# arpg/Kangaroo

Measured on AMD Instinct MI355X. Metric: kinectfusion_frames_per_sec_640x480_to_512cubed_tsdf, higher is better.
Workload: dtype f32

## Files before the change

kangaroo_amd/csrc/kfx_device.h:

```cpp
#pragma once

#include <hip/hip_runtime.h>
#include <stddef.h>
#include <stdint.h>

#include "../../include/kfx.h"
#include "../../include/kfx_extras.h"
#include "../../include/kfx_summary_h.h"
#include "../../include/kfx_color.h"
#include "summary_ring_host.h"

namespace kfx {

struct V3 { float x, y, z; };

__device__ __forceinline__ V3 v3(float x, float y, float z) { return V3{x, y, z}; }
__device__ __forceinline__ V3 operator+(V3 a, V3 b) { return V3{a.x + b.x, a.y + b.y, a.z + b.z}; }
__device__ __forceinline__ V3 operator-(V3 a, V3 b) { return V3{a.x - b.x, a.y - b.y, a.z - b.z}; }
__device__ __forceinline__ V3 operator*(V3 a, float s) { return V3{a.x * s, a.y * s, a.z * s}; }
__device__ __forceinline__ V3 div_cw(V3 a, V3 b) { return V3{a.x / b.x, a.y / b.y, a.z / b.z}; }
__device__ __forceinline__ V3 div_s(V3 a, float s) { const float inv = 1.0f / s; return a * inv; }
__device__ __forceinline__ float dot(V3 a, V3 b) { return a.x * b.x + a.y * b.y + a.z * b.z; }
__device__ __forceinline__ float length(V3 a) { return sqrtf(dot(a, a)); }
__device__ __forceinline__ float lerp(float a, float b, float t) { return a + t * (b - a); }
// ... 224 lines not shown
                all_either = all_either && c != 0;
            }
            cls = all_free ? 1 : (all_nan ? 2 : (all_either ? 3 : 0));
        }
        const unsigned long long p0 = __ballot(cls & 1), p1 = __ballot(cls & 2);
        if (e < total && (bx & 63) == 0 && (chunks > 1 || bx == 0)) {
            const int sh = chunks > 1 ? 0 : lane;
            const unsigned long long m = (chunks > 1 || lg == 6) ? ~0ull : ((1ull << (1 << lg)) - 1ull);
            const unsigned long long r0 = (p0 >> sh) & m, r1 = (p1 >> sh) & m;
            unsigned* out = tab + dst.first + (bz * dst.ny + by) * dst.rw + (bx >> 6) * 4;
            out[0] = (unsigned)r0; out[1] = (unsigned)r1;
            if ((bx >> 6) * 4 + 2 < dst.rw) { out[2] = (unsigned)(r0 >> 32); out[3] = (unsigned)(r1 >> 32); }
        }
    }
}
int summary_classes_prepare(kfx_sdf_summary* s, float tol, float vref, int fine_shift, hipStream_t stream, int global = 0);
void summary_class_layout(const kfx_sdf_summary* s, int fine_shift, ClassView& cv);
void summary_top_layout(const ClassView& cv, ClassLevel& l6, ClassLevel& l7, int& w6, int& w7);
int summary_view_offset(const kfx_sdf_summary* s, const kfx_volume* view, int* ox, int* oy, int* oz);
}

namespace kfx {
int set_error(int code, const char* what);
int check_launch(const char* what);
int hip_status(hipError_t e, const char* what);
int math_mode();
size_t texel_image_bytes(size_t w, size_t h);
int depth_to_vbo_normals_texels(const kfx_image* vbo, const kfx_image* nrm, const kfx_image* depth, const float K[4], float scale,
                                const kfx_image* texels, kfx_stream stream);
int sdf_fuse_slab_texels(const kfx_volume* vol, const kfx_slab* slab, const kfx_image* depth, const kfx_image* norm, const kfx_image* texels,
                         const float T_cw[12], const float K[4], float trunc_dist, float max_w, float mincostheta, unsigned flags, kfx_stream stream);
// ... 4 lines not shown
```

kangaroo_amd/csrc/raycast.hip:

```cpp
#include <cmath>
#include <thread>

#include <hip/hip_fp16.h>

#include "kfx_device.h"
#include "sampling.h"
#include "../../include/kfx_slab_color.h"

namespace kfx {

struct RayParams {
    VolView vol;
    V3 size;
    V3 dims1;
    V3 hi2;
    V3 voxel;
    V3 inv_size;
    int fastdiv, off32;
    Pose T;
    Intr K;
    unsigned char *dptr, *nptr, *iptr;
    size_t dpitch, npitch, ipitch;
    int w, h;
    float near, far, trunc;
// ... 353 lines not shown
    const int at = GT ? 0 : cl.words;
    class_level_up(cl.nx5, cl.coarse.ny, cl.nz5, 6, at, l6, nx6, nz6, w6);
    class_level_up(nx6, l6.ny, nz6, 7, at + w6, l7, nx7, nz7, w7);
    if (threadIdx.x == 0) { top.lv[0] = l6; top.lv[1] = l7; top.n = cl.top_n; }
    __syncthreads();
}

__device__ __forceinline__ bool workgroup_any(const bool yes, int* s_any)
{
    const bool wave_any = __ballot(yes) != 0ull;
    if ((threadIdx.x & 63) == 0) s_any[threadIdx.x >> 6] = wave_any ? 1 : 0;
    __syncthreads();
    return (s_any[0] | s_any[1] | s_any[2] | s_any[3]) != 0;
}

template <typename CELL, bool GT = false>
__global__ __launch_bounds__(256) void k_raycast_sdf_classes(const RayParams p, const ClassView cl)
{
    extern __shared__ unsigned s_tab[];
    __shared__ RayParams s_p;
    __shared__ TopLevels s_top;
    __shared__ int s_any[4];
    if (threadIdx.x == 0) s_p = p;
    int u, v;
    const bool carries = ray_lane_pixel(p, p.sparse_lanes, blockIdx.x, blockIdx.y, u, v);
    const bool pixel = carries && u < p.w && v < p.h;
    if constexpr (!GT) {
        if (!workgroup_any(pixel && enters(ray_box(p, u, v)), s_any)) {
            if (pixel) write_no_hit(ray_out(p, u, v));
            return;
        }
    }
    classes_stage<GT>(cl, s_tab, s_top);
    if (!carries) return;
    raycast_pixel_classes<CELL, false, false, GT>(p, s_p, ColorGeom{}, u, v, cl, s_tab, s_top);
}

template <typename CELL, bool COLOR>
__global__ __launch_bounds__(256) void k_raycast_sdf(const RayParams p, const ColorGeom cv)
{
    int u, v;
    if (!ray_lane_pixel(p, p.sparse_lanes, blockIdx.x, blockIdx.y, u, v)) return;
    raycast_pixel<CELL, COLOR>(p, cv, u, v);
}

template <typename CELL>
__global__ __launch_bounds__(256) void k_raycast_sdf_count(const RayParams p, unsigned* __restrict__ bitmap, unsigned long long* __restrict__ counters)
{
    int u, v;
    ray_pixel_of(p, blockIdx.x, blockIdx.y, threadIdx.x, u, v);
// ... 305 lines not shown
    p.npitch = norm->pitch;
    p.ipitch = img->pitch;
    p.w = (int)img->w;
    p.h = (int)img->h;
    p.near = near;
    p.far = far;
    p.trunc = trunc_dist;
    p.subpix = subpix ? 1 : 0;
    p.tile_log2w = 5;
    p.wg_log2x = 1;
    p.sparse_lanes = 0;
    return 0;
}

template <typename CELL>
static int class_view(ClassView& cl, size_t* lds_bytes, int* usable, kfx_sdf_summary* summary, const kfx_volume* vol, const RayParams& p, kfx_stream stream,
                      bool allow_global = true)
{
    *usable = 0;
    if (int e = summary_view_offset(summary, vol, &cl.ox, &cl.oy, &cl.oz)) return e;
    if (!(p.trunc > 0.f) || !(p.trunc < __builtin_inff())) return 0;
    static const int kb_env = env_int("KFX_RAYCAST_CLASS_KB", 16, 1, 60);
    static const int gt_env = env_int("KFX_RAYCAST_GLOBAL_TABLES", 0);
    static const int top_env = env_int("KFX_RAYCAST_TOP_LEVELS", 2, 0, 2);
    int fine = 3;
    for (; fine < 5; ++fine) {
        summary_class_layout(summary, fine, cl);
        if ((size_t)cl.words * 4 <= (size_t)kb_env * 1024) break;
    }
    auto top_levels = [&](int& w6, int& w7) {
        summary_class_layout(summary, fine, cl);
        cl.nx5 = ceil_div(summary->w, 32); cl.nz5 = ceil_div(summary->d, 32);
        ClassLevel l6, l7;
        summary_top_layout(cl, l6, l7, w6, w7);
// ... 14 lines not shown
        cl.top_first = cl.words;
        cl.lds_words = (cl.top_n > 0 ? w6 : 0) + (cl.top_n > 1 ? w7 : 0);
        if ((size_t)cl.lds_words * 4 + lds_static > 64 * 1024) return 0;
    } else {
        cl.top_first = 0;
        cl.lds_words = cl.words + derived;
    }
    if (cl.global && !allow_global) return 0;
    const bool half = CELL::BYTES == 4;
    const float vref = half ? __half2float(__float2half_rn(p.trunc)) : p.trunc;
    const float tol = math_mode() == KFX_MATH_FAST ? (half ? KFX_SUMMARY_HALF_BAND : 1e-5f) : 0.f;
    static const int force_env = env_int("KFX_RAYCAST_SUMMARY", 0);
    if (force_env < 0) return 0;
    const bool steer = force_env == 0 && summary->h_skippable;
    if (steer && summary->plain_calls && (summary->plain_calls++ % 8u) != 0u) return 0;
    if (int e = summary_classes_prepare(summary, tol, vref, fine, (hipStream_t)stream, cl.global)) return e;
    if (steer && summary->builds >= 3) {
        const unsigned ref = summary->builds - 3;
        const unsigned long long* slot = summary->h_skippable + summary_ring_index(ref);
        int known = 0;
        const int seen = summary_ring_wait(
            ref, 1ull << 20,
            [&]() {
                const uint64_t v = __atomic_load_n(slot, __ATOMIC_ACQUIRE);
                if (summary_ring_slot_stamp(v) != summary_ring_stamp(ref)) std::this_thread::yield();
                return v;
            },
            [&]() { (void)hipStreamSynchronize((hipStream_t)stream); }, &known);
        if (seen < 0) return set_error(KFX_E_TIMEOUT, "RaycastSdf(tracked): the class-table build the choice of the march rests on has not published its count");
        if ((long long)known * 4 < summary->n_coarse) {
            if (!summary->plain_calls) summary->plain_calls = 1;
// ... 13 lines not shown
    for (int a = 0; a < 3; ++a) {
        if (!(size[a] > 0.f)) return 0;
        const double sc = (double)dims1[a] / size[a];
        const double pmax = std::fmax(std::fabs((double)bmin[a]), std::fabs((double)bmax[a])), ca = std::fabs((double)cw[a]);
        const double A = std::fabs(((double)cw[a] - bmin[a]) * sc);
        const double t = sc * (3.0 * pmax + 2.0 * ca + size[a]) * u24 + 2.0 * dims1[a] * u24;
        const double e = u24 * (3.0 * A + 2.0 * sc * (pmax + ca) + dims1[a]) + 3.0 * u24 * (dims1[a] + A);
        eps = std::fmax(eps, t + e);
    }
    eps *= 2.0;
    if (!(eps < 0.05)) return 0;
    cl.eps = (float)std::fmax(eps, 1e-4);
    *lds_bytes = (size_t)cl.lds_words * sizeof(unsigned);
    *usable = 1;
    return 0;
}

template <typename PLAIN, typename... A>
static int launch_march(const char* what, int usable, const ClassView& cl, size_t cl_bytes, dim3 grid, kfx_stream stream, const RayParams& p,
                        void (*global)(RayParams, ClassView, A...), void (*lds)(RayParams, ClassView, A...), PLAIN plain, A... a)
{
    if (usable) hipLaunchKernelGGL(cl.global ? global : lds, grid, dim3(256), cl_bytes, (hipStream_t)stream, p, cl, a...);
    else plain();
    return check_launch(what);
}

template <typename CELL>
static int raycast_levels_launch(int n_levels, const kfx_image* const* depth, const kfx_image* const* norm, const kfx_image* const* img,
                                 const kfx_image* const* vbo, const kfx_volume* vol, const float T_wc[12], const float* K, float near, float far,
                                 float trunc_dist, int subpix, kfx_stream stream, kfx_sdf_summary* summary = nullptr)
// ... 64 lines not shown
    static const int lanes_env = [] { const int v = env_int("KFX_RAYCAST_LANES", 0); return (v == 8 || v == 16 || v == 32) ? v : (v < 0 ? -1 : 0); }();
    const int lanes = lanes_env ? lanes_env : ((long long)p.w * p.h <= 160 * 120 ? 16 : 0);
    if (lanes && lanes_env >= 0) {
        p.sparse_lanes = lanes;
        grid = dim3(ceil_div(p.w, 2 * lanes), ceil_div(p.h, 2));
    }
    ColorGeom cv{};
    if (colorvol) {
        if (int e = check_volume(colorvol, 4, 2, VOLUME_ANY_DIM, "RaycastSdf(colour)")) return e;
        set_geometry(cv, colorvol);
        hipLaunchKernelGGL((k_raycast_sdf<CELL, true>), grid, dim3(256), 0, (hipStream_t)stream, p, cv);
    } else if (summary) {
        ClassView cl;
        size_t cl_bytes = 0;
        int usable = 0;
        if (int e = class_view<CELL>(cl, &cl_bytes, &usable, summary, vol, p, stream)) return e;
        return launch_march("kfx_raycast_sdf_tracked", usable, cl, cl_bytes, grid, stream, p, k_raycast_sdf_classes<CELL, true>, k_raycast_sdf_classes<CELL, false>,
                            [&] { hipLaunchKernelGGL((k_raycast_sdf<CELL, false>), grid, dim3(256), 0, (hipStream_t)stream, p, cv); });
    } else {
        hipLaunchKernelGGL((k_raycast_sdf<CELL, false>), grid, dim3(256), 0, (hipStream_t)stream, p, cv);
    }
    return check_launch("kfx_raycast_sdf");
}

extern "C" int kfx_raycast_sdf(const kfx_image* depth, const kfx_image* norm, const kfx_image* img,
                               const kfx_volume* vol, const float T_wc[12], const float K[4], float near,
                               float far, float trunc_dist, int subpix, kfx_stream stream)
{
    return raycast_launch<RayF32>(depth, norm, img, vol, T_wc, K, near, far, trunc_dist, subpix, stream);
}

template <typename CELL>
static int count_params(RayParams& p, dim3& grid, const kfx_volume* vol, unsigned w, unsigned h, const float T_wc[12], const float K[4], float near, float far,
// ... 307 lines not shown
```

kangaroo_amd/csrc/summary.hip:

```cpp
#include <algorithm>
#include <new>

#include <hip/hip_fp16.h>

#include "kfx_device.h"

namespace kfx {

__global__ __launch_bounds__(256) void k_summary_fill(float4* __restrict__ R, size_t n, float lo, float hi, int state)
{
    const size_t i = (size_t)blockIdx.x * 256 + threadIdx.x;
    if (i < n) R[i] = make_float4(lo, hi, __int_as_float(state), 0.f);
}

struct ClassBuild {
    const float4* R;
    unsigned* C;
    int nbx, nby, nbz;
    int shift, nx, ny, nz, rw;
    float lo_ok, hi_ok;
    const unsigned* src;
    int src_shift, src_nx, src_ny, src_nz, src_rw;
};
struct TopBuild {
    int on;
    unsigned* tab;
    ClassLevel l5, l6, l7;
    int nx5, nz5, nx6, nz6, nx7, nz7;
};
template <int M>
__device__ __forceinline__ int class_row(const ClassBuild& b, const long long wave)
{
    const float4* __restrict__ R = b.R;
    unsigned* __restrict__ C = b.C;
    const unsigned* __restrict__ src = b.src;
    const int nbx = b.nbx, nby = b.nby, nbz = b.nbz, shift = b.shift, nx = b.nx, ny = b.ny, rw = b.rw;
    const int src_shift = b.src_shift, src_nx = b.src_nx, src_ny = b.src_ny, src_nz = b.src_nz, src_rw = b.src_rw;
    const float lo_ok = b.lo_ok, hi_ok = b.hi_ok;
    const int lane = threadIdx.x & 63;
    const int chunks = (nx + 63) >> 6;
    const int chunk = (int)(wave % chunks), by = (int)((wave / chunks) % ny), bz = (int)(wave / ((long long)chunks * ny));
    const int bx = chunk * 64 + lane;
    int cls = 0;
    if (bx < nx) {
        bool all_nan = true, all_free = true, all_either = true;
        if constexpr (M == 0) {
            const int m = 1 << (shift - src_shift);
            for (int z0 = 0; z0 < m; z0 += 2) {
                uint2 w2[2][4];
#pragma unroll
                for (int dz = 0; dz < 2; ++dz)
#pragma unroll
                    for (int dy = 0; dy < 4; ++dy) {
                        const int z = min(bz * m + z0 + dz, src_nz - 1), y = min(by * m + min(dy, m - 1), src_ny - 1);
                        w2[dz][dy] = *reinterpret_cast<const uint2*>(src + ((size_t)z * src_ny + y) * src_rw + (((bx * m) >> 5) << 1));
                    }
#pragma unroll
                for (int dz = 0; dz < 2; ++dz)
#pragma unroll
                    for (int dy = 0; dy < 4; ++dy)
                        for (int dx = 0; dx < m; ++dx) {
                            const int x = min(bx * m + dx, src_nx - 1);
                            const int c = (int)((w2[dz][dy].x >> (x & 31)) & 1u) | (int)(((w2[dz][dy].y >> (x & 31)) & 1u) << 1);
                            all_free = all_free && c == 1;
                            all_nan = all_nan && c == 2;
                            all_either = all_either && c != 0;
                        }
            }
        } else if constexpr (M > 2) {
#pragma unroll 1
            for (int z = bz * M; z <= bz * M + M; ++z)
#pragma unroll 1
                for (int y = by * M; y <= by * M + M; ++y) {
                    const float4* __restrict__ Rrow = R + ((size_t)min(z, nbz - 1) * nby + min(y, nby - 1)) * nbx;
                    float4 r[M + 1];
#pragma unroll
                    for (int dx = 0; dx <= M; ++dx) r[dx] = Rrow[min(bx * M + dx, nbx - 1)];
#pragma unroll
                    for (int dx = 0; dx <= M; ++dx) {
                        const unsigned m = brick_class_mask(r[dx].x, r[dx].y, __float_as_int(r[dx].z), lo_ok, hi_ok);
                        all_nan = all_nan && (m & 1u);
                        all_free = all_free && (m & 2u);
                        all_either = all_either && (m & 4u);
                    }
                }
        } else {
            float4 r[(M + 1) * (M + 1) * (M + 1)];
#pragma unroll
            for (int dz = 0; dz <= M; ++dz)
#pragma unroll
                for (int dy = 0; dy <= M; ++dy)
#pragma unroll
                    for (int dx = 0; dx <= M; ++dx)
                        r[(dz * (M + 1) + dy) * (M + 1) + dx] =
                            R[((size_t)min(bz * M + dz, nbz - 1) * nby + min(by * M + dy, nby - 1)) * nbx + min(bx * M + dx, nbx - 1)];
#pragma unroll
            for (int k = 0; k < (M + 1) * (M + 1) * (M + 1); ++k) {
                const unsigned m = brick_class_mask(r[k].x, r[k].y, __float_as_int(r[k].z), lo_ok, hi_ok);
                all_nan = all_nan && (m & 1u);
                all_free = all_free && (m & 2u);
                all_either = all_either && (m & 4u);
            }
        }
        cls = all_free ? 1 : (all_nan ? 2 : (all_either ? 3 : 0));
    }
    const unsigned long long p0 = __ballot(cls & 1), p1 = __ballot(cls & 2);
    if (lane == 0) {
        unsigned* row = C + ((size_t)bz * ny + by) * rw + chunk * 4;
        row[0] = (unsigned)p0; row[1] = (unsigned)p1;
        if (chunk * 4 + 2 < rw) { row[2] = (unsigned)(p0 >> 32); row[3] = (unsigned)(p1 >> 32); }
    }
    return __popcll(p0 | p1);
}

__device__ __forceinline__ bool classes_up_to_date(int* __restrict__ count, unsigned long long* __restrict__ publish, const unsigned stamp,
                                                   const int* __restrict__ dirty, const int conditional)
{
    if (!conditional || *dirty != 0) return false;
    if (blockIdx.x == 0 && threadIdx.x == 0) {
        __hip_atomic_store(publish, ((unsigned long long)stamp << 32) | (unsigned)count[2], __ATOMIC_RELAXED, __HIP_MEMORY_SCOPE_SYSTEM);
        count[4] += 1;
    }
    return true;
}

__device__ __forceinline__ void classes_count_and_top(const int n, int* __restrict__ count, unsigned long long* __restrict__ publish, const unsigned stamp,
                                                      int* __restrict__ dirty, const int conditional, const TopBuild& t)
{
    __shared__ int s_count[4];
    __shared__ int s_last;
    if ((threadIdx.x & 63) == 0) s_count[threadIdx.x >> 6] = n;
    __threadfence();
    __syncthreads();
    if (threadIdx.x == 0) {
        s_last = 0;
        atomicAdd(&count[0], s_count[0] + s_count[1] + s_count[2] + s_count[3]);
        __threadfence();
        if (atomicAdd(&count[1], 1) == (int)gridDim.x - 1) {
            __threadfence();
            s_last = 1;
            const int total = atomicExch(&count[0], 0);
            count[1] = 0;
            count[2] = total;
            if (conditional) count[3] += 1;
            *dirty = 0;
            __hip_atomic_store(publish, ((unsigned long long)stamp << 32) | (unsigned)total, __ATOMIC_RELAXED, __HIP_MEMORY_SCOPE_SYSTEM);
        }
    }
    __syncthreads();
    if (t.on && s_last) {
        __threadfence();
        classes_level_up(t.tab, t.l5, t.nx5, t.nz5, t.l6, t.nx6, t.nz6);
        __threadfence();
        __syncthreads();
        classes_level_up(t.tab, t.l6, t.nx6, t.nz6, t.l7, t.nx7, t.nz7);
    }
}

struct FineRows {
    unsigned* C;
    int shift, nx, ny, nz, rw;
    int blocks;
    long long waves;
};
template <int MF>
__global__ __launch_bounds__(256) void k_summary_classes_build(const FineRows f, const ClassBuild c, const long long c_waves, int* __restrict__ count,
                                                               unsigned long long* __restrict__ publish, const unsigned stamp, int* __restrict__ dirty,
                                                               const int conditional, const TopBuild t)
{
    if (classes_up_to_date(count, publish, stamp, dirty, conditional)) return;
    int n = 0;
    bool fine_row = false;
    if constexpr (MF != 0) {
        fine_row = (int)blockIdx.x < f.blocks;
        if (fine_row) {
            ClassBuild b = c;
            b.C = f.C; b.shift = f.shift; b.nx = f.nx; b.ny = f.ny; b.nz = f.nz; b.rw = f.rw;
            const long long wave = (long long)blockIdx.x * 4 + (threadIdx.x >> 6);
            if (wave < f.waves) class_row<MF>(b, wave);
        }
    }
    if (!fine_row) {
        const long long wave = (long long)((int)blockIdx.x - f.blocks) * 4 + (threadIdx.x >> 6);
        if (wave < c_waves) n = class_row<4>(c, wave);
    }
    classes_count_and_top(n, count, publish, stamp, dirty, conditional, t);
}

template <int M>
__global__ __launch_bounds__(256) void k_summary_classes(const ClassBuild b, const long long n_waves)
{
    const long long wave = (long long)blockIdx.x * 4 + (threadIdx.x >> 6);
    if (wave < n_waves) class_row<M>(b, wave);
}

__global__ __launch_bounds__(256) void k_summary_classes_coarse(const ClassBuild b, const long long n_waves, int* __restrict__ count,
                                                                unsigned long long* __restrict__ publish, const unsigned stamp, int* __restrict__ dirty, const TopBuild t)
{
    const long long wave = (long long)blockIdx.x * 4 + (threadIdx.x >> 6);
    const int n = wave < n_waves ? class_row<0>(b, wave) : 0;
    classes_count_and_top(n, count, publish, stamp, dirty, 0, t);
}

template <int BYTES>
__global__ __launch_bounds__(256) void k_summary_rebuild(float4* __restrict__ R, const unsigned char* __restrict__ base, size_t pitch, size_t img_pitch,
                                                         int w, int h, int d, int nbx, int nby, int nbz, int aligned16)
{
    const long long brick = (long long)blockIdx.x * 4 + (threadIdx.x >> 6);
    if (brick >= (long long)nbx * nby * nbz) return;
    const int lane = threadIdx.x & 63;
    const int bx = (int)(brick % nbx), by = (int)((brick / nbx) % nby), bz = (int)(brick / ((long long)nbx * nby));
    const int y = by * 8 + (lane & 7), z = bz * 8 + (lane >> 3), x0 = bx * 8;
    float lo = __builtin_inff(), hi = -__builtin_inff();
    bool nan = false, val = false;
    if (y < h && z < d) {
        const unsigned char* row = base + (size_t)z * img_pitch + (size_t)y * pitch + (size_t)x0 * BYTES;
// ... 61 lines not shown
void summary_class_layout(const kfx_sdf_summary* s, int fine_shift, ClassView& cv)
{
    class_level(cv.fine, fine_shift, s->w, s->h, 0);
    const int fw = fine_shift < 5 ? class_level_words(cv.fine, s->d) : 0;
    class_level(cv.coarse, 5, s->w, s->h, (fw + 3) & ~3);
    cv.words = cv.coarse.first + ((class_level_words(cv.coarse, s->d) + 3) & ~3);
}

void summary_top_layout(const ClassView& cv, ClassLevel& l6, ClassLevel& l7, int& w6, int& w7)
{
    int nx6, nz6, nx7, nz7;
    class_level_up(cv.nx5, cv.coarse.ny, cv.nz5, 6, cv.words, l6, nx6, nz6, w6);
    class_level_up(nx6, l6.ny, nz6, 7, cv.words + w6, l7, nx7, nz7, w7);
}

int summary_classes_prepare(kfx_sdf_summary* s, float tol, float vref, int fine_shift, hipStream_t stream, int global)
{
    const bool same = s->c_tol == tol && s->c_vref == vref && s->c_shift == fine_shift && s->c_global == global;
    if (!s->c_dirty && same) return 0;
    const int conditional = (s->c_dirty == 1 && same && !global) ? 1 : 0;
    ClassView cv;
    summary_class_layout(s, fine_shift, cv);
    cv.nx5 = ceil_div(s->w, 32); cv.nz5 = ceil_div(s->d, 32);
    ClassLevel l6, l7;
    int w6, w7;
    summary_top_layout(cv, l6, l7, w6, w7);
    TopBuild top{};
    top.on = global ? 0 : 1;
    top.tab = s->C;
    top.l5 = cv.coarse; top.l6 = l6; top.l7 = l7;
    top.nx5 = cv.nx5; top.nz5 = cv.nz5;
    top.nx6 = (top.nx5 + 1) >> 1; top.nz6 = (top.nz5 + 1) >> 1;
// ... 19 lines not shown
    if (global && has_fine) {
        const ClassBuild f = level(cv.fine, nullptr), c = level(cv.coarse, &cv.fine);
        if (cv.fine.shift == 3) hipLaunchKernelGGL(k_summary_classes<1>, dim3(blocks_of(f)), dim3(256), 0, stream, f, waves_of(f));
        else hipLaunchKernelGGL(k_summary_classes<2>, dim3(blocks_of(f)), dim3(256), 0, stream, f, waves_of(f));
        if (int e = launched()) return e;
        hipLaunchKernelGGL(k_summary_classes_coarse, dim3(blocks_of(c)), dim3(256), 0, stream, c, waves_of(c), s->d_count, publish, stamp, s->d_dirty, top);
        if (int e = launched()) return e;
    } else {
        const ClassBuild c = level(cv.coarse, nullptr);
        FineRows f{};
        if (has_fine) {
            const ClassBuild b = level(cv.fine, nullptr);
            f.C = b.C; f.shift = b.shift; f.nx = b.nx; f.ny = b.ny; f.nz = b.nz; f.rw = b.rw;
            f.blocks = (int)blocks_of(b); f.waves = waves_of(b);
        }
        const dim3 grid((unsigned)f.blocks + blocks_of(c));
        if (!has_fine) hipLaunchKernelGGL(k_summary_classes_build<0>, grid, dim3(256), 0, stream, f, c, waves_of(c), s->d_count, publish, stamp, s->d_dirty, conditional, top);
        else if (cv.fine.shift == 3) hipLaunchKernelGGL(k_summary_classes_build<1>, grid, dim3(256), 0, stream, f, c, waves_of(c), s->d_count, publish, stamp, s->d_dirty, conditional, top);
        else hipLaunchKernelGGL(k_summary_classes_build<2>, grid, dim3(256), 0, stream, f, c, waves_of(c), s->d_count, publish, stamp, s->d_dirty, conditional, top);
        if (int e = launched()) return e;
    }
    s->builds += 1;
    if (global) {
        for (int up = 0; up < 2; ++up) {
            const ClassBuild b = level(up ? l7 : l6, up ? &l6 : &cv.coarse);
            hipLaunchKernelGGL(k_summary_classes<0>, dim3(blocks_of(b)), dim3(256), 0, stream, b, waves_of(b));
            if (int e = launched()) return e;
        }
    }
    s->c_dirty = 0; s->c_tol = tol; s->c_vref = vref; s->c_shift = fine_shift; s->c_global = global;
    s->c_lo_ok = lo_ok; s->c_hi_ok = hi_ok;
    return 0;
}

int summary_view_offset(const kfx_sdf_summary* s, const kfx_volume* view, int* ox, int* oy, int* oz)
// ... 31 lines not shown
    s->keep_stride = 0; s->keep_row0 = 0; s->keep_rows = 0;
    s->c_lo_ok = 0.f; s->c_hi_ok = 0.f; s->d_dirty = nullptr;
    s->builds = 0; s->plain_calls = 0; s->launches = 0;
    s->n_coarse = ceil_div(s->w, 32) * ceil_div(s->h, 32) * ceil_div(s->d, 32);
    const size_t n = (size_t)s->nbx * s->nby * s->nbz;
    ClassView cv;
    summary_class_layout(s, 3, cv);
    cv.nx5 = ceil_div(s->w, 32); cv.nz5 = ceil_div(s->d, 32);
    ClassLevel l6, l7;
    int w6, w7;
    summary_top_layout(cv, l6, l7, w6, w7);
    const int words = cv.words + w6 + w7;
    bool ok = hipMalloc((void**)&s->R, n * sizeof(float4)) == hipSuccess && hipMalloc((void**)&s->C, (size_t)words * sizeof(unsigned)) == hipSuccess &&
              hipMalloc((void**)&s->d_count, 64 * sizeof(int)) == hipSuccess && hipMemset(s->d_count, 0, 64 * sizeof(int)) == hipSuccess;
    if (ok) s->d_dirty = s->d_count + 32;
    if (ok && hipHostMalloc((void**)&s->h_skippable, KFX_SUMMARY_RING * sizeof(unsigned long long), hipHostMallocMapped) == hipSuccess) {
        for (int i = 0; i < KFX_SUMMARY_RING; ++i) s->h_skippable[i] = 0ull;
        if (hipHostGetDevicePointer((void**)&s->d_skippable, s->h_skippable, 0) != hipSuccess) {
            (void)hipHostFree(s->h_skippable);
            s->h_skippable = nullptr;
        }
    } else {
        s->h_skippable = nullptr;
    }
    if (ok && !s->h_skippable) {
        (void)hipGetLastError();
        ok = hipMalloc((void**)&s->d_skippable, sizeof(unsigned long long)) == hipSuccess;
    }
    if (!ok) {
        (void)hipGetLastError();
        kfx_sdf_summary_destroy(s);
        return set_error(KFX_E_NODEVICE, "kfx_sdf_summary_create: hipMalloc");
    }
    *out = s;
    return kfx_sdf_summary_invalidate(s, nullptr);
}

extern "C" int kfx_sdf_summary_create(kfx_sdf_summary** out, const kfx_volume* vol) { return summary_create(out, vol, 8); }
extern "C" int kfx_sdf_summary_create_h(kfx_sdf_summary** out, const kfx_volume* vol) { return summary_create(out, vol, 4); }

extern "C" int kfx_sdf_summary_destroy(kfx_sdf_summary* s)
{
    if (!s) return 0;
    (void)hipDeviceSynchronize();
    if (s->R) (void)hipFree(s->R);
    if (s->C) (void)hipFree(s->C);
    if (s->d_count) (void)hipFree(s->d_count);
    if (s->h_skippable) (void)hipHostFree(s->h_skippable);
    else if (s->d_skippable) (void)hipFree(s->d_skippable);
    delete s;
    return 0;
}

extern "C" int kfx_sdf_summary_rebuild(kfx_sdf_summary* s, kfx_stream stream)
{
    if (!s) return set_error(KFX_E_NULL, "kfx_sdf_summary_rebuild: null summary");
    const long long n = (long long)s->nbx * s->nby * s->nbz;
    const int aligned16 = ((((uintptr_t)s->base) | s->pitch | s->img_pitch) & 15) == 0;
    if (s->cell_bytes == 4)
        hipLaunchKernelGGL(k_summary_rebuild<4>, dim3((unsigned)((n + 3) / 4)), dim3(256), 0, (hipStream_t)stream, s->R, s->base, s->pitch, s->img_pitch,
                           s->w, s->h, s->d, s->nbx, s->nby, s->nbz, aligned16);
    else
        hipLaunchKernelGGL(k_summary_rebuild<8>, dim3((unsigned)((n + 3) / 4)), dim3(256), 0, (hipStream_t)stream, s->R, s->base, s->pitch, s->img_pitch,
                           s->w, s->h, s->d, s->nbx, s->nby, s->nbz, aligned16);
    s->c_dirty = 2;
    return check_launch("kfx_sdf_summary_rebuild");
}

extern "C" int kfx_sdf_summary_invalidate(kfx_sdf_summary* s, kfx_stream stream)
{
    if (!s) return set_error(KFX_E_NULL, "kfx_sdf_summary_invalidate: null summary");
    const size_t n = (size_t)s->nbx * s->nby * s->nbz;
    hipLaunchKernelGGL(k_summary_fill, dim3((unsigned)((n + 255) / 256)), dim3(256), 0, (hipStream_t)stream, s->R, n, -__builtin_inff(), __builtin_inff(), 2);
    s->c_dirty = 2;
    return check_launch("kfx_sdf_summary_invalidate");
}

static int reset_tracked(const kfx_volume* vol, kfx_sdf_summary* s, float trunc_dist, kfx_stream stream, int cell_bytes, const char* name)
{
    if (!s) return set_error(KFX_E_NULL, cell_bytes == 4 ? "kfx_sdf_reset_tracked_h: null summary" : "kfx_sdf_reset_tracked: null summary");
    if (s->cell_bytes != cell_bytes) return set_error(KFX_E_SHAPE, "SdfReset(tracked): the summary was created for the other cell type");
    int ox, oy, oz;
    if (int e = summary_view_offset(s, vol, &ox, &oy, &oz)) return e;
    if (ox || oy || oz || (int)vol->w != s->w || (int)vol->h != s->h || (int)vol->d != s->d)
        return set_error(KFX_E_SHAPE, "kfx_sdf_reset_tracked: resets the whole volume only (use kfx_sdf_reset + kfx_sdf_summary_invalidate for views)");
    if (int e = cell_bytes == 4 ? kfx_sdf_reset_h(vol, trunc_dist, stream) : kfx_sdf_reset(vol, trunc_dist, stream)) return e;
    const size_t n = (size_t)s->nbx * s->nby * s->nbz;
    const bool nan = trunc_dist != trunc_dist;
    const float v = cell_bytes == 4 ? __half2float(__float2half_rn(trunc_dist)) : trunc_dist;
    hipLaunchKernelGGL(k_summary_fill, dim3((unsigned)((n + 255) / 256)), dim3(256), 0, (hipStream_t)stream, s->R, n,
                       nan ? __builtin_inff() : v, nan ? -__builtin_inff() : v, nan ? 1 : 0);
    s->c_dirty = 2;
    return check_launch(name);
}

extern "C" int kfx_sdf_reset_tracked(const kfx_volume* vol, kfx_sdf_summary* s, float trunc_dist, kfx_stream stream)
// ... 9 lines not shown
```

Measured before the change: 2637.

## Fuse class-table build into the tracked raycast launch via ticketed work-sharing

```diff
diff --git a/kangaroo_amd/csrc/kfx_device.h b/kangaroo_amd/csrc/kfx_device.h
--- a/kangaroo_amd/csrc/kfx_device.h
+++ b/kangaroo_amd/csrc/kfx_device.h
@@ -262,7 +262,10 @@
         }
     }
 }
-int summary_classes_prepare(kfx_sdf_summary* s, float tol, float vref, int fine_shift, hipStream_t stream, int global = 0);
+struct ClassRide;
+int summary_classes_prepare(kfx_sdf_summary* s, float tol, float vref, int fine_shift, hipStream_t stream, int global = 0, ClassRide* ride = nullptr);
+int summary_classes_launch(kfx_sdf_summary* s, const ClassRide& b, int conditional, hipStream_t stream, bool counted);
+int summary_ride_error(kfx_sdf_summary* s);
 void summary_class_layout(const kfx_sdf_summary* s, int fine_shift, ClassView& cv);
 void summary_top_layout(const ClassView& cv, ClassLevel& l6, ClassLevel& l7, int& w6, int& w7);
 int summary_view_offset(const kfx_sdf_summary* s, const kfx_volume* view, int* ox, int* oy, int* oz);
diff --git a/kangaroo_amd/csrc/raycast.hip b/kangaroo_amd/csrc/raycast.hip
--- a/kangaroo_amd/csrc/raycast.hip
+++ b/kangaroo_amd/csrc/raycast.hip
@@ -4,6 +4,7 @@
 #include <hip/hip_fp16.h>
 
 #include "kfx_device.h"
+#include "summary_build.h"
 #include "sampling.h"
 #include "../../include/kfx_slab_color.h"
 
@@ -391,13 +392,18 @@
     return (s_any[0] | s_any[1] | s_any[2] | s_any[3]) != 0;
 }
 
-template <typename CELL, bool GT = false>
-__global__ __launch_bounds__(256) void k_raycast_sdf_classes(const RayParams p, const ClassView cl)
-{
-    extern __shared__ unsigned s_tab[];
-    __shared__ RayParams s_p;
-    __shared__ TopLevels s_top;
-    __shared__ int s_any[4];
+struct ClassesArgs { RayParams p; ClassView cl; ClassRide rb; };
+typedef const __attribute__((address_space(4))) ClassesArgs* ClassesArgsPtr;
+__device__ __forceinline__ ClassesArgsPtr classes_args()
+{
+    ClassesArgsPtr a = (ClassesArgsPtr)__builtin_amdgcn_kernarg_segment_ptr();
+    asm volatile("" : "+s"(a));
+    return a;
+}
+
+template <typename CELL, bool GT>
+__device__ __forceinline__ void march_classes(const RayParams& p, const ClassView& cl, unsigned* s_tab, RayParams& s_p, TopLevels& s_top, int* s_any)
+{
     if (threadIdx.x == 0) s_p = p;
     int u, v;
     const bool carries = ray_lane_pixel(p, p.sparse_lanes, blockIdx.x, blockIdx.y, u, v);
@@ -411,6 +417,37 @@
     classes_stage<GT>(cl, s_tab, s_top);
     if (!carries) return;
     raycast_pixel_classes<CELL, false, false, GT>(p, s_p, ColorGeom{}, u, v, cl, s_tab, s_top);
+}
+
+template <typename CELL, bool GT = false>
+__global__ __launch_bounds__(256) void k_raycast_sdf_classes(const RayParams p, const ClassView cl, const ClassRide rb)
+{
+    extern __shared__ unsigned s_tab[];
+    __shared__ RayParams s_p;
+    __shared__ TopLevels s_top;
+    __shared__ int s_any[4];
+    if constexpr (GT) {
+        march_classes<CELL, true>(p, cl, s_tab, s_p, s_top, s_any);
+    } else {
+        if (rb.on) {
+            __shared__ int s_ride[2];
+            const int d = __builtin_amdgcn_readfirstlane(__hip_atomic_load(rb.dirty, __ATOMIC_RELAXED, __HIP_MEMORY_SCOPE_AGENT));
+            if (d == CLASSES_DIRTY || d == classes_built_mark(rb.stamp)) {
+                ClassesArgsPtr a = classes_args();
+                if (!classes_ride(*(const ClassRide*)&a->rb, s_ride)) {
+                    const RayParams& q = *(const RayParams*)&a->p;
+                    int u, v;
+                    if (ray_lane_pixel(q, q.sparse_lanes, blockIdx.x, blockIdx.y, u, v)) raycast_pixel<CELL, false>(q, ColorGeom{}, u, v);
+                    return;
+                }
+            } else if (blockIdx.x == 0 && blockIdx.y == 0 && threadIdx.x == 0) {
+                ClassesArgsPtr a = classes_args();
+                classes_publish_retained(a->rb.count, a->rb.publish, rb.stamp);
+            }
+        }
+        ClassesArgsPtr a = classes_args();
+        march_classes<CELL, false>(*(const RayParams*)&a->p, *(const ClassView*)&a->cl, s_tab, s_p, s_top, s_any);
+    }
 }
 
 template <typename CELL, bool COLOR>
@@ -746,10 +783,11 @@
 }
 
 template <typename CELL>
-static int class_view(ClassView& cl, size_t* lds_bytes, int* usable, kfx_sdf_summary* summary, const kfx_volume* vol, const RayParams& p, kfx_stream stream,
-                      bool allow_global = true)
+static int class_view_tables(ClassView& cl, size_t* lds_bytes, int* usable, kfx_sdf_summary* summary, const kfx_volume* vol, const RayParams& p, kfx_stream stream,
+                             bool allow_global, ClassRide* ride)
 {
     *usable = 0;
+    if (int e = summary_ride_error(summary)) return e;
     if (int e = summary_view_offset(summary, vol, &cl.ox, &cl.oy, &cl.oz)) return e;
     if (!(p.trunc > 0.f) || !(p.trunc < __builtin_inff())) return 0;
     static const int kb_env = env_int("KFX_RAYCAST_CLASS_KB", 16, 1, 60);
@@ -794,7 +832,7 @@
     if (force_env < 0) return 0;
     const bool steer = force_env == 0 && summary->h_skippable;
     if (steer && summary->plain_calls && (summary->plain_calls++ % 8u) != 0u) return 0;
-    if (int e = summary_classes_prepare(summary, tol, vref, fine, (hipStream_t)stream, cl.global)) return e;
+    if (int e = summary_classes_prepare(summary, tol, vref, fine, (hipStream_t)stream, cl.global, ride)) return e;
     if (steer && summary->builds >= 3) {
         const unsigned ref = summary->builds - 3;
         const unsigned long long* slot = summary->h_skippable + summary_ring_index(ref);
@@ -838,6 +876,19 @@
     *lds_bytes = (size_t)cl.lds_words * sizeof(unsigned);
     *usable = 1;
     return 0;
+}
+
+template <typename CELL>
+static int class_view(ClassView& cl, size_t* lds_bytes, int* usable, kfx_sdf_summary* summary, const kfx_volume* vol, const RayParams& p, kfx_stream stream,
+                      bool allow_global = true, ClassRide* ride = nullptr)
+{
+    const int e = class_view_tables<CELL>(cl, lds_bytes, usable, summary, vol, p, stream, allow_global, ride);
+    if (ride && ride->on && (e || !*usable || cl.global)) {
+        ride->on = 0;
+        const int le = summary_classes_launch(summary, *ride, 1, (hipStream_t)stream, true);
+        return e ? e : le;
+    }
+    return e;
 }
 
 template <typename PLAIN, typename... A>
@@ -932,9 +983,10 @@
         ClassView cl;
         size_t cl_bytes = 0;
         int usable = 0;
-        if (int e = class_view<CELL>(cl, &cl_bytes, &usable, summary, vol, p, stream)) return e;
+        ClassRide ride{};
+        if (int e = class_view<CELL>(cl, &cl_bytes, &usable, summary, vol, p, stream, true, &ride)) return e;
         return launch_march("kfx_raycast_sdf_tracked", usable, cl, cl_bytes, grid, stream, p, k_raycast_sdf_classes<CELL, true>, k_raycast_sdf_classes<CELL, false>,
-                            [&] { hipLaunchKernelGGL((k_raycast_sdf<CELL, false>), grid, dim3(256), 0, (hipStream_t)stream, p, cv); });
+                            [&] { hipLaunchKernelGGL((k_raycast_sdf<CELL, false>), grid, dim3(256), 0, (hipStream_t)stream, p, cv); }, ride);
     } else {
         hipLaunchKernelGGL((k_raycast_sdf<CELL, false>), grid, dim3(256), 0, (hipStream_t)stream, p, cv);
     }
diff --git a/kangaroo_amd/csrc/summary.hip b/kangaroo_amd/csrc/summary.hip
--- a/kangaroo_amd/csrc/summary.hip
+++ b/kangaroo_amd/csrc/summary.hip
@@ -4,6 +4,7 @@
 #include <hip/hip_fp16.h>
 
 #include "kfx_device.h"
+#include "summary_build.h"
 
 namespace kfx {
 
@@ -13,178 +14,14 @@
     if (i < n) R[i] = make_float4(lo, hi, __int_as_float(state), 0.f);
 }
 
-struct ClassBuild {
-    const float4* R;
-    unsigned* C;
-    int nbx, nby, nbz;
-    int shift, nx, ny, nz, rw;
-    float lo_ok, hi_ok;
-    const unsigned* src;
-    int src_shift, src_nx, src_ny, src_nz, src_rw;
-};
-struct TopBuild {
-    int on;
-    unsigned* tab;
-    ClassLevel l5, l6, l7;
-    int nx5, nz5, nx6, nz6, nx7, nz7;
-};
-template <int M>
-__device__ __forceinline__ int class_row(const ClassBuild& b, const long long wave)
-{
-    const float4* __restrict__ R = b.R;
-    unsigned* __restrict__ C = b.C;
-    const unsigned* __restrict__ src = b.src;
-    const int nbx = b.nbx, nby = b.nby, nbz = b.nbz, shift = b.shift, nx = b.nx, ny = b.ny, rw = b.rw;
-    const int src_shift = b.src_shift, src_nx = b.src_nx, src_ny = b.src_ny, src_nz = b.src_nz, src_rw = b.src_rw;
-    const float lo_ok = b.lo_ok, hi_ok = b.hi_ok;
-    const int lane = threadIdx.x & 63;
-    const int chunks = (nx + 63) >> 6;
-    const int chunk = (int)(wave % chunks), by = (int)((wave / chunks) % ny), bz = (int)(wave / ((long long)chunks * ny));
-    const int bx = chunk * 64 + lane;
-    int cls = 0;
-    if (bx < nx) {
-        bool all_nan = true, all_free = true, all_either = true;
-        if constexpr (M == 0) {
-            const int m = 1 << (shift - src_shift);
-            for (int z0 = 0; z0 < m; z0 += 2) {
-                uint2 w2[2][4];
-#pragma unroll
-                for (int dz = 0; dz < 2; ++dz)
-#pragma unroll
-                    for (int dy = 0; dy < 4; ++dy) {
-                        const int z = min(bz * m + z0 + dz, src_nz - 1), y = min(by * m + min(dy, m - 1), src_ny - 1);
-                        w2[dz][dy] = *reinterpret_cast<const uint2*>(src + ((size_t)z * src_ny + y) * src_rw + (((bx * m) >> 5) << 1));
-                    }
-#pragma unroll
-                for (int dz = 0; dz < 2; ++dz)
-#pragma unroll
-                    for (int dy = 0; dy < 4; ++dy)
-                        for (int dx = 0; dx < m; ++dx) {
-                            const int x = min(bx * m + dx, src_nx - 1);
-                            const int c = (int)((w2[dz][dy].x >> (x & 31)) & 1u) | (int)(((w2[dz][dy].y >> (x & 31)) & 1u) << 1);
-                            all_free = all_free && c == 1;
-                            all_nan = all_nan && c == 2;
-                            all_either = all_either && c != 0;
-                        }
-            }
-        } else if constexpr (M > 2) {
-#pragma unroll 1
-            for (int z = bz * M; z <= bz * M + M; ++z)
-#pragma unroll 1
-                for (int y = by * M; y <= by * M + M; ++y) {
-                    const float4* __restrict__ Rrow = R + ((size_t)min(z, nbz - 1) * nby + min(y, nby - 1)) * nbx;
-                    float4 r[M + 1];
-#pragma unroll
-                    for (int dx = 0; dx <= M; ++dx) r[dx] = Rrow[min(bx * M + dx, nbx - 1)];
-#pragma unroll
-                    for (int dx = 0; dx <= M; ++dx) {
-                        const unsigned m = brick_class_mask(r[dx].x, r[dx].y, __float_as_int(r[dx].z), lo_ok, hi_ok);
-                        all_nan = all_nan && (m & 1u);
-                        all_free = all_free && (m & 2u);
-                        all_either = all_either && (m & 4u);
-                    }
-                }
-        } else {
-            float4 r[(M + 1) * (M + 1) * (M + 1)];
-#pragma unroll
-            for (int dz = 0; dz <= M; ++dz)
-#pragma unroll
-                for (int dy = 0; dy <= M; ++dy)
-#pragma unroll
-                    for (int dx = 0; dx <= M; ++dx)
-                        r[(dz * (M + 1) + dy) * (M + 1) + dx] =
-                            R[((size_t)min(bz * M + dz, nbz - 1) * nby + min(by * M + dy, nby - 1)) * nbx + min(bx * M + dx, nbx - 1)];
-#pragma unroll
-            for (int k = 0; k < (M + 1) * (M + 1) * (M + 1); ++k) {
-                const unsigned m = brick_class_mask(r[k].x, r[k].y, __float_as_int(r[k].z), lo_ok, hi_ok);
-                all_nan = all_nan && (m & 1u);
-                all_free = all_free && (m & 2u);
-                all_either = all_either && (m & 4u);
-            }
-        }
-        cls = all_free ? 1 : (all_nan ? 2 : (all_either ? 3 : 0));
-    }
-    const unsigned long long p0 = __ballot(cls & 1), p1 = __ballot(cls & 2);
-    if (lane == 0) {
-        unsigned* row = C + ((size_t)bz * ny + by) * rw + chunk * 4;
-        row[0] = (unsigned)p0; row[1] = (unsigned)p1;
-        if (chunk * 4 + 2 < rw) { row[2] = (unsigned)(p0 >> 32); row[3] = (unsigned)(p1 >> 32); }
-    }
-    return __popcll(p0 | p1);
-}
-
-__device__ __forceinline__ bool classes_up_to_date(int* __restrict__ count, unsigned long long* __restrict__ publish, const unsigned stamp,
-                                                   const int* __restrict__ dirty, const int conditional)
-{
-    if (!conditional || *dirty != 0) return false;
-    if (blockIdx.x == 0 && threadIdx.x == 0) {
-        __hip_atomic_store(publish, ((unsigned long long)stamp << 32) | (unsigned)count[2], __ATOMIC_RELAXED, __HIP_MEMORY_SCOPE_SYSTEM);
-        count[4] += 1;
-    }
-    return true;
-}
-
-__device__ __forceinline__ void classes_count_and_top(const int n, int* __restrict__ count, unsigned long long* __restrict__ publish, const unsigned stamp,
-                                                      int* __restrict__ dirty, const int conditional, const TopBuild& t)
-{
-    __shared__ int s_count[4];
-    __shared__ int s_last;
-    if ((threadIdx.x & 63) == 0) s_count[threadIdx.x >> 6] = n;
-    __threadfence();
-    __syncthreads();
-    if (threadIdx.x == 0) {
-        s_last = 0;
-        atomicAdd(&count[0], s_count[0] + s_count[1] + s_count[2] + s_count[3]);
-        __threadfence();
-        if (atomicAdd(&count[1], 1) == (int)gridDim.x - 1) {
-            __threadfence();
-            s_last = 1;
-            const int total = atomicExch(&count[0], 0);
-            count[1] = 0;
-            count[2] = total;
-            if (conditional) count[3] += 1;
-            *dirty = 0;
-            __hip_atomic_store(publish, ((unsigned long long)stamp << 32) | (unsigned)total, __ATOMIC_RELAXED, __HIP_MEMORY_SCOPE_SYSTEM);
-        }
-    }
-    __syncthreads();
-    if (t.on && s_last) {
-        __threadfence();
-        classes_level_up(t.tab, t.l5, t.nx5, t.nz5, t.l6, t.nx6, t.nz6);
-        __threadfence();
-        __syncthreads();
-        classes_level_up(t.tab, t.l6, t.nx6, t.nz6, t.l7, t.nx7, t.nz7);
-    }
-}
-
-struct FineRows {
-    unsigned* C;
-    int shift, nx, ny, nz, rw;
-    int blocks;
-    long long waves;
-};
 template <int MF>
 __global__ __launch_bounds__(256) void k_summary_classes_build(const FineRows f, const ClassBuild c, const long long c_waves, int* __restrict__ count,
                                                                unsigned long long* __restrict__ publish, const unsigned stamp, int* __restrict__ dirty,
                                                                const int conditional, const TopBuild t)
 {
     if (classes_up_to_date(count, publish, stamp, dirty, conditional)) return;
-    int n = 0;
-    bool fine_row = false;
-    if constexpr (MF != 0) {
-        fine_row = (int)blockIdx.x < f.blocks;
-        if (fine_row) {
-            ClassBuild b = c;
-            b.C = f.C; b.shift = f.shift; b.nx = f.nx; b.ny = f.ny; b.nz = f.nz; b.rw = f.rw;
-            const long long wave = (long long)blockIdx.x * 4 + (threadIdx.x >> 6);
-            if (wave < f.waves) class_row<MF>(b, wave);
-        }
-    }
-    if (!fine_row) {
-        const long long wave = (long long)((int)blockIdx.x - f.blocks) * 4 + (threadIdx.x >> 6);
-        if (wave < c_waves) n = class_row<4>(c, wave);
-    }
-    classes_count_and_top(n, count, publish, stamp, dirty, conditional, t);
+    const int n = classes_share<MF>(f, c, c_waves, (int)blockIdx.x);
+    classes_count_and_top(n, count, publish, stamp, dirty, conditional, t, (int)gridDim.x, 0);
 }
 
 template <int M>
@@ -199,7 +36,7 @@
 {
     const long long wave = (long long)blockIdx.x * 4 + (threadIdx.x >> 6);
     const int n = wave < n_waves ? class_row<0>(b, wave) : 0;
-    classes_count_and_top(n, count, publish, stamp, dirty, 0, t);
+    classes_count_and_top(n, count, publish, stamp, dirty, 0, t, (int)gridDim.x, 0);
 }
 
 template <int BYTES>
@@ -291,8 +128,28 @@
     class_level_up(nx6, l6.ny, nz6, 7, cv.words + w6, l7, nx7, nz7, w7);
 }
 
-int summary_classes_prepare(kfx_sdf_summary* s, float tol, float vref, int fine_shift, hipStream_t stream, int global)
-{
+int summary_classes_launch(kfx_sdf_summary* s, const ClassRide& b, int conditional, hipStream_t stream, bool counted)
+{
+    const dim3 grid((unsigned)b.shares);
+    if (b.mf == 0) hipLaunchKernelGGL(k_summary_classes_build<0>, grid, dim3(256), 0, stream, b.f, b.c, b.c_waves, b.count, b.publish, b.stamp, b.dirty, conditional, b.t);
+    else if (b.mf == 1) hipLaunchKernelGGL(k_summary_classes_build<1>, grid, dim3(256), 0, stream, b.f, b.c, b.c_waves, b.count, b.publish, b.stamp, b.dirty, conditional, b.t);
+    else hipLaunchKernelGGL(k_summary_classes_build<2>, grid, dim3(256), 0, stream, b.f, b.c, b.c_waves, b.count, b.publish, b.stamp, b.dirty, conditional, b.t);
+    if (!counted) s->launches += 1;
+    return check_launch("kfx_sdf_summary (classes)");
+}
+
+int summary_ride_error(kfx_sdf_summary* s)
+{
+    if (!s->h_skippable) return 0;
+    const uint64_t v = __atomic_exchange_n(s->h_skippable + KFX_SUMMARY_RING, 0ull, __ATOMIC_ACQ_REL);
+    if (!v) return 0;
+    s->c_dirty = 2;
+    return set_error(KFX_E_TIMEOUT, "kfx_sdf_summary: a class-table build inside a RaycastSdf(tracked) launch did not complete in time; that launch marched plainly");
+}
+
+int summary_classes_prepare(kfx_sdf_summary* s, float tol, float vref, int fine_shift, hipStream_t stream, int global, ClassRide* ride)
+{
+    if (ride) ride->on = 0;
     const bool same = s->c_tol == tol && s->c_vref == vref && s->c_shift == fine_shift && s->c_global == global;
     if (!s->c_dirty && same) return 0;
     const int conditional = (s->c_dirty == 1 && same && !global) ? 1 : 0;
@@ -342,11 +199,21 @@
             f.C = b.C; f.shift = b.shift; f.nx = b.nx; f.ny = b.ny; f.nz = b.nz; f.rw = b.rw;
             f.blocks = (int)blocks_of(b); f.waves = waves_of(b);
         }
-        const dim3 grid((unsigned)f.blocks + blocks_of(c));
-        if (!has_fine) hipLaunchKernelGGL(k_summary_classes_build<0>, grid, dim3(256), 0, stream, f, c, waves_of(c), s->d_count, publish, stamp, s->d_dirty, conditional, top);
-        else if (cv.fine.shift == 3) hipLaunchKernelGGL(k_summary_classes_build<1>, grid, dim3(256), 0, stream, f, c, waves_of(c), s->d_count, publish, stamp, s->d_dirty, conditional, top);
-        else hipLaunchKernelGGL(k_summary_classes_build<2>, grid, dim3(256), 0, stream, f, c, waves_of(c), s->d_count, publish, stamp, s->d_dirty, conditional, top);
-        if (int e = launched()) return e;
+        ClassRide b{};
+        b.mf = !has_fine ? 0 : (cv.fine.shift == 3 ? 1 : 2);
+        b.shares = f.blocks + (int)blocks_of(c);
+        b.stamp = stamp;
+        b.f = f; b.c = c; b.c_waves = waves_of(c); b.t = top;
+        b.count = s->d_count; b.publish = publish; b.dirty = s->d_dirty;
+        b.tickets = reinterpret_cast<unsigned long long*>(s->d_count + 8);
+        b.error = s->d_skippable + (s->h_skippable ? KFX_SUMMARY_RING : 1);
+        if (conditional && ride) {
+            b.on = 1;
+            *ride = b;
+            s->launches += 1;
+        } else {
+            if (int e = summary_classes_launch(s, b, conditional, stream, false)) return e;
+        }
     }
     s->builds += 1;
     if (global) {
@@ -408,8 +275,8 @@
     bool ok = hipMalloc((void**)&s->R, n * sizeof(float4)) == hipSuccess && hipMalloc((void**)&s->C, (size_t)words * sizeof(unsigned)) == hipSuccess &&
               hipMalloc((void**)&s->d_count, 64 * sizeof(int)) == hipSuccess && hipMemset(s->d_count, 0, 64 * sizeof(int)) == hipSuccess;
     if (ok) s->d_dirty = s->d_count + 32;
-    if (ok && hipHostMalloc((void**)&s->h_skippable, KFX_SUMMARY_RING * sizeof(unsigned long long), hipHostMallocMapped) == hipSuccess) {
-        for (int i = 0; i < KFX_SUMMARY_RING; ++i) s->h_skippable[i] = 0ull;
+    if (ok && hipHostMalloc((void**)&s->h_skippable, (KFX_SUMMARY_RING + 1) * sizeof(unsigned long long), hipHostMallocMapped) == hipSuccess) {
+        for (int i = 0; i <= KFX_SUMMARY_RING; ++i) s->h_skippable[i] = 0ull;
         if (hipHostGetDevicePointer((void**)&s->d_skippable, s->h_skippable, 0) != hipSuccess) {
             (void)hipHostFree(s->h_skippable);
             s->h_skippable = nullptr;
@@ -419,7 +286,7 @@
     }
     if (ok && !s->h_skippable) {
         (void)hipGetLastError();
-        ok = hipMalloc((void**)&s->d_skippable, sizeof(unsigned long long)) == hipSuccess;
+        ok = hipMalloc((void**)&s->d_skippable, 2 * sizeof(unsigned long long)) == hipSuccess;
     }
     if (!ok) {
         (void)hipGetLastError();
@@ -449,6 +316,7 @@
 extern "C" int kfx_sdf_summary_rebuild(kfx_sdf_summary* s, kfx_stream stream)
 {
     if (!s) return set_error(KFX_E_NULL, "kfx_sdf_summary_rebuild: null summary");
+    if (int e = summary_ride_error(s)) return e;
     const long long n = (long long)s->nbx * s->nby * s->nbz;
     const int aligned16 = ((((uintptr_t)s->base) | s->pitch | s->img_pitch) & 15) == 0;
     if (s->cell_bytes == 4)
@@ -464,6 +332,7 @@
 extern "C" int kfx_sdf_summary_invalidate(kfx_sdf_summary* s, kfx_stream stream)
 {
     if (!s) return set_error(KFX_E_NULL, "kfx_sdf_summary_invalidate: null summary");
+    if (int e = summary_ride_error(s)) return e;
     const size_t n = (size_t)s->nbx * s->nby * s->nbz;
     hipLaunchKernelGGL(k_summary_fill, dim3((unsigned)((n + 255) / 256)), dim3(256), 0, (hipStream_t)stream, s->R, n, -__builtin_inff(), __builtin_inff(), 2);
     s->c_dirty = 2;
@@ -474,6 +343,7 @@
 {
     if (!s) return set_error(KFX_E_NULL, cell_bytes == 4 ? "kfx_sdf_reset_tracked_h: null summary" : "kfx_sdf_reset_tracked: null summary");
     if (s->cell_bytes != cell_bytes) return set_error(KFX_E_SHAPE, "SdfReset(tracked): the summary was created for the other cell type");
+    if (int e = summary_ride_error(s)) return e;
     int ox, oy, oz;
     if (int e = summary_view_offset(s, vol, &ox, &oy, &oz)) return e;
     if (ox || oy || oz || (int)vol->w != s->w || (int)vol->h != s->h || (int)vol->d != s->d)
diff --git a/kangaroo_amd/csrc/summary_build.h b/kangaroo_amd/csrc/summary_build.h
--- /dev/null
+++ b/kangaroo_amd/csrc/summary_build.h
@@ -0,0 +1,258 @@
+#pragma once
+#include "kfx_device.h"
+
+namespace kfx {
+
+struct ClassBuild {
+    const float4* R;
+    unsigned* C;
+    int nbx, nby, nbz;
+    int shift, nx, ny, nz, rw;
+    float lo_ok, hi_ok;
+    const unsigned* src;
+    int src_shift, src_nx, src_ny, src_nz, src_rw;
+};
+struct TopBuild {
+    int on;
+    unsigned* tab;
+    ClassLevel l5, l6, l7;
+    int nx5, nz5, nx6, nz6, nx7, nz7;
+};
+struct FineRows {
+    unsigned* C;
+    int shift, nx, ny, nz, rw;
+    int blocks;
+    long long waves;
+};
+
+template <int M, bool ROLLED = false>
+__device__ __forceinline__ int class_row(const ClassBuild& b, const long long wave)
+{
+    const float4* __restrict__ R = b.R;
+    unsigned* __restrict__ C = b.C;
+    const unsigned* __restrict__ src = b.src;
+    const int nbx = b.nbx, nby = b.nby, nbz = b.nbz, shift = b.shift, nx = b.nx, ny = b.ny, rw = b.rw;
+    const int src_shift = b.src_shift, src_nx = b.src_nx, src_ny = b.src_ny, src_nz = b.src_nz, src_rw = b.src_rw;
+    const float lo_ok = b.lo_ok, hi_ok = b.hi_ok;
+    const int lane = threadIdx.x & 63;
+    const int chunks = (nx + 63) >> 6;
+    const int chunk = (int)(wave % chunks), by = (int)((wave / chunks) % ny), bz = (int)(wave / ((long long)chunks * ny));
+    const int bx = chunk * 64 + lane;
+    int cls = 0;
+    if (bx < nx) {
+        bool all_nan = true, all_free = true, all_either = true;
+        if constexpr (M == 0) {
+            const int m = 1 << (shift - src_shift);
+            for (int z0 = 0; z0 < m; z0 += 2) {
+                uint2 w2[2][4];
+#pragma unroll
+                for (int dz = 0; dz < 2; ++dz)
+#pragma unroll
+                    for (int dy = 0; dy < 4; ++dy) {
+                        const int z = min(bz * m + z0 + dz, src_nz - 1), y = min(by * m + min(dy, m - 1), src_ny - 1);
+                        w2[dz][dy] = *reinterpret_cast<const uint2*>(src + ((size_t)z * src_ny + y) * src_rw + (((bx * m) >> 5) << 1));
+                    }
+#pragma unroll
+                for (int dz = 0; dz < 2; ++dz)
+#pragma unroll
+                    for (int dy = 0; dy < 4; ++dy)
+                        for (int dx = 0; dx < m; ++dx) {
+                            const int x = min(bx * m + dx, src_nx - 1);
+                            const int c = (int)((w2[dz][dy].x >> (x & 31)) & 1u) | (int)(((w2[dz][dy].y >> (x & 31)) & 1u) << 1);
+                            all_free = all_free && c == 1;
+                            all_nan = all_nan && c == 2;
+                            all_either = all_either && c != 0;
+                        }
+            }
+        } else if constexpr (M > 2 || ROLLED) {
+#pragma unroll 1
+            for (int z = bz * M; z <= bz * M + M; ++z)
+#pragma unroll 1
+                for (int y = by * M; y <= by * M + M; ++y) {
+                    const float4* __restrict__ Rrow = R + ((size_t)min(z, nbz - 1) * nby + min(y, nby - 1)) * nbx;
+                    float4 r[M + 1];
+#pragma unroll
+                    for (int dx = 0; dx <= M; ++dx) r[dx] = Rrow[min(bx * M + dx, nbx - 1)];
+#pragma unroll
+                    for (int dx = 0; dx <= M; ++dx) {
+                        const unsigned m = brick_class_mask(r[dx].x, r[dx].y, __float_as_int(r[dx].z), lo_ok, hi_ok);
+                        all_nan = all_nan && (m & 1u);
+                        all_free = all_free && (m & 2u);
+                        all_either = all_either && (m & 4u);
+                    }
+                }
+        } else {
+            float4 r[(M + 1) * (M + 1) * (M + 1)];
+#pragma unroll
+            for (int dz = 0; dz <= M; ++dz)
+#pragma unroll
+                for (int dy = 0; dy <= M; ++dy)
+#pragma unroll
+                    for (int dx = 0; dx <= M; ++dx)
+                        r[(dz * (M + 1) + dy) * (M + 1) + dx] =
+                            R[((size_t)min(bz * M + dz, nbz - 1) * nby + min(by * M + dy, nby - 1)) * nbx + min(bx * M + dx, nbx - 1)];
+#pragma unroll
+            for (int k = 0; k < (M + 1) * (M + 1) * (M + 1); ++k) {
+                const unsigned m = brick_class_mask(r[k].x, r[k].y, __float_as_int(r[k].z), lo_ok, hi_ok);
+                all_nan = all_nan && (m & 1u);
+                all_free = all_free && (m & 2u);
+                all_either = all_either && (m & 4u);
+            }
+        }
+        cls = all_free ? 1 : (all_nan ? 2 : (all_either ? 3 : 0));
+    }
+    const unsigned long long p0 = __ballot(cls & 1), p1 = __ballot(cls & 2);
+    if (lane == 0) {
+        unsigned* row = C + ((size_t)bz * ny + by) * rw + chunk * 4;
+        row[0] = (unsigned)p0; row[1] = (unsigned)p1;
+        if (chunk * 4 + 2 < rw) { row[2] = (unsigned)(p0 >> 32); row[3] = (unsigned)(p1 >> 32); }
+    }
+    return __popcll(p0 | p1);
+}
+
+template <int MF, bool ROLLED = false>
+__device__ __forceinline__ int classes_share(const FineRows& f, const ClassBuild& c, const long long c_waves, const int share)
+{
+    int n = 0;
+    bool fine_row = false;
+    if constexpr (MF != 0) {
+        fine_row = share < f.blocks;
+        if (fine_row) {
+            ClassBuild b = c;
+            b.C = f.C; b.shift = f.shift; b.nx = f.nx; b.ny = f.ny; b.nz = f.nz; b.rw = f.rw;
+            const long long wave = (long long)share * 4 + (threadIdx.x >> 6);
+            if (wave < f.waves) class_row<MF, ROLLED>(b, wave);
+        }
+    }
+    if (!fine_row) {
+        const long long wave = (long long)(share - f.blocks) * 4 + (threadIdx.x >> 6);
+        if (wave < c_waves) n = class_row<4>(c, wave);
+    }
+    return n;
+}
+
+constexpr int CLASSES_DIRTY = 1;
+__host__ __device__ inline int classes_built_mark(const unsigned stamp) { return (int)(0x80000000u | stamp); }
+
+__device__ __forceinline__ int classes_first_thread()
+{
+    int zero = 0;
+    asm volatile("" : "+v"(zero));
+    return zero;
+}
+
+__device__ __forceinline__ void classes_publish_retained(int* __restrict__ count, unsigned long long* __restrict__ publish, const unsigned stamp)
+{
+    __hip_atomic_store(publish, ((unsigned long long)stamp << 32) | (unsigned)count[2], __ATOMIC_RELAXED, __HIP_MEMORY_SCOPE_SYSTEM);
+    count[4] += 1;
+}
+
+__device__ __forceinline__ bool classes_up_to_date(int* __restrict__ count, unsigned long long* __restrict__ publish, const unsigned stamp,
+                                                   const int* __restrict__ dirty, const int conditional)
+{
+    if (!conditional || *dirty == CLASSES_DIRTY) return false;
+    if (blockIdx.x == 0 && threadIdx.x == 0) classes_publish_retained(count, publish, stamp);
+    return true;
+}
+
+__device__ __forceinline__ bool classes_count_and_top(const int n, int* __restrict__ count, unsigned long long* __restrict__ publish, const unsigned stamp,
+                                                      int* __restrict__ dirty, const int conditional, const TopBuild& t, const int parts, const int done)
+{
+    __shared__ int s_count[4];
+    __shared__ int s_last;
+    if ((threadIdx.x & 63) == 0) s_count[threadIdx.x >> 6] = n;
+    __threadfence();
+    __syncthreads();
+    if ((int)threadIdx.x == classes_first_thread()) {
+        s_last = 0;
+        atomicAdd(&count[0], s_count[0] + s_count[1] + s_count[2] + s_count[3]);
+        __threadfence();
+        if (atomicAdd(&count[1], 1) == parts - 1) {
+            __threadfence();
+            s_last = 1;
+            const int total = atomicExch(&count[0], 0);
+            count[1] = 0;
+            count[2] = total;
+            if (conditional) count[3] += 1;
+            __hip_atomic_store(publish, ((unsigned long long)stamp << 32) | (unsigned)total, __ATOMIC_RELAXED, __HIP_MEMORY_SCOPE_SYSTEM);
+        }
+    }
+    __syncthreads();
+    const bool last = __builtin_amdgcn_readfirstlane(s_last) != 0;
+    if (last) {
+        if (t.on) {
+            __threadfence();
+            classes_level_up(t.tab, t.l5, t.nx5, t.nz5, t.l6, t.nx6, t.nz6);
+            __threadfence();
+            __syncthreads();
+            classes_level_up(t.tab, t.l6, t.nx6, t.nz6, t.l7, t.nx7, t.nz7);
+        }
+        __threadfence();
+        __syncthreads();
+        if (threadIdx.x == 0) __hip_atomic_store(dirty, done, __ATOMIC_RELEASE, __HIP_MEMORY_SCOPE_AGENT);
+    }
+    return last;
+}
+
+struct ClassRide {
+    int on;
+    unsigned stamp;
+    int* dirty;
+    int mf;
+    int shares;
+    FineRows f;
+    ClassBuild c;
+    long long c_waves;
+    TopBuild t;
+    int* count;
+    unsigned long long* publish;
+    unsigned long long* tickets;
+    unsigned long long* error;
+};
+
+constexpr int CLASSES_RIDE_POLLS = 1 << 16;
+
+__device__ __forceinline__ int classes_ticket(unsigned long long* tickets, const unsigned stamp)
+{
+    for (;;) {
+        const unsigned long long old = __hip_atomic_fetch_add(tickets, 1ull, __ATOMIC_RELAXED, __HIP_MEMORY_SCOPE_AGENT);
+        if ((unsigned)(old >> 32) == stamp) return (int)(unsigned)old;
+        unsigned long long seen = old + 1ull;
+        while ((unsigned)(seen >> 32) != stamp &&
+               !__hip_atomic_compare_exchange_strong(tickets, &seen, (unsigned long long)stamp << 32, __ATOMIC_RELAXED, __ATOMIC_RELAXED,
+                                                     __HIP_MEMORY_SCOPE_AGENT)) {
+        }
+    }
+}
+
+__device__ __forceinline__ bool classes_ride(const ClassRide& rb, int* s_w)
+{
+    const int mark = classes_built_mark(rb.stamp);
+    for (;;) {
+        if ((int)threadIdx.x == classes_first_thread()) s_w[0] = classes_ticket(rb.tickets, rb.stamp);
+        __syncthreads();
+        const int share = __builtin_amdgcn_readfirstlane(s_w[0]);
+        __syncthreads();
+        if (share >= rb.shares) break;
+        int n;
+        if (rb.mf == 2) n = classes_share<2, true>(rb.f, rb.c, rb.c_waves, share);
+        else if (rb.mf == 1) n = classes_share<1, true>(rb.f, rb.c, rb.c_waves, share);
+        else n = classes_share<0>(rb.f, rb.c, rb.c_waves, share);
+        classes_count_and_top(n, rb.count, rb.publish, rb.stamp, rb.dirty, 1, rb.t, rb.shares, mark);
+    }
+    if (threadIdx.x == 0) {
+        int ok = 0;
+        for (int i = 0; i < CLASSES_RIDE_POLLS && !ok; ++i) {
+            ok = __hip_atomic_load(rb.dirty, __ATOMIC_RELAXED, __HIP_MEMORY_SCOPE_AGENT) == mark ? 1 : 0;
+            if (!ok) __builtin_amdgcn_s_sleep(16);
+        }
+        if (!ok) __hip_atomic_store(rb.error, 1ull, __ATOMIC_RELAXED, __HIP_MEMORY_SCOPE_SYSTEM);
+        s_w[1] = ok;
+    }
+    __syncthreads();
+    if (!__builtin_amdgcn_readfirstlane(s_w[1])) return false;
+    __threadfence();
+    return true;
+}
+
+}
```

New measurement: 2649 (median of 6 runs). No clear change (+0.4%).
